# xin-pu/yolo-continuous

Measured on AMD Instinct MI355X. Metric: images/sec (whole node) + p50 end-to-end latency, 640×640 bs=32, 1/2/4/8 MI355X, higher is better.
Workload: dtype bf16; 1 GPU; yolov7 COCO-80 640x640, 32 images per GPU per step: forward + decode + NMS (+ all-gather); global_batch=32, per_gpu_batch=32, image_size=640, parallelism=dp1, hip_graph=True, mode=concurrent, batches_in_flight=3, max_det=300

## Files before the change

yolo-continuous_amd/csrc/ycx_misc.hip:

```cpp
#include <dlfcn.h>
#include <stdio.h>
#include <vector>

#include "ycx_internal.h"

namespace {

template <typename T>
struct Vec;
template <>
struct Vec<__bf16> {
  typedef bf16x8 type;
  static constexpr int N = 8;
};
template <>
struct Vec<_Float16> {
  typedef __attribute__((ext_vector_type(8))) _Float16 type;
  static constexpr int N = 8;
};
template <>
struct Vec<float> {
  typedef f32x4 type;
  static constexpr int N = 4;
};

template <typename T>
__global__ void __launch_bounds__(256) maxpool_kernel(ycx_pool_desc d, const T* __restrict__ x,
                                                      T* __restrict__ y) {
  typedef typename Vec<T>::type V;
  constexpr int VN = Vec<T>::N;
  const int cv = d.c / VN;
  const long long total = (long long)d.n * d.ho * d.wo * cv;
  for (long long i = blockIdx.x * (long long)blockDim.x + threadIdx.x; i < total;
       i += (long long)gridDim.x * blockDim.x) {
    int c = (int)(i % cv);
    long long p = i / cv;
    int ox = (int)(p % d.wo);
    long long t = p / d.wo;
    int oy = (int)(t % d.ho);
    int n = (int)(t / d.ho);
    float m[VN];
#pragma unroll
    for (int j = 0; j < VN; ++j) m[j] = -INFINITY;
    const int y0 = oy * d.stride - d.pad, x0 = ox * d.stride - d.pad;
    const int ya = max(y0, 0), yb = min(y0 + d.k, d.h), xa = max(x0, 0), xb = min(x0 + d.k, d.w);
    for (int iy = ya; iy < yb; ++iy)
      for (int ix = xa; ix < xb; ++ix) {
        V v = *reinterpret_cast<const V*>(x + (((size_t)n * d.h + iy) * d.w + ix) * d.in_c_stride +
                                          d.in_c_off + c * VN);
#pragma unroll
        for (int j = 0; j < VN; ++j) m[j] = ycx_pool_max(m[j], (float)v[j]);
      }
    V o;
#pragma unroll
    for (int j = 0; j < VN; ++j) o[j] = (T)m[j];
    *reinterpret_cast<V*>(y + (((size_t)n * d.ho + oy) * d.wo + ox) * d.out_c_stride + d.out_c_off +
                          c * VN) = o;
  }
}

template <typename T>
__global__ void __launch_bounds__(256) maxpool_rows_kernel(ycx_pool_desc d, const T* __restrict__ x,
                                                           T* __restrict__ y) {
  typedef typename Vec<T>::type V;
  constexpr int VN = Vec<T>::N;
  const int cv = d.c / VN;
  const int i = blockIdx.x * blockDim.x + threadIdx.x;
  if (i >= d.wo * cv) return;
  const int row = blockIdx.y, n = row / d.ho, oy = row - n * d.ho;
  const int ox = i / cv, c = i - ox * cv;
  float m[VN];
#pragma unroll
  for (int j = 0; j < VN; ++j) m[j] = -INFINITY;
  const int y0 = oy * d.stride - d.pad, x0 = ox * d.stride - d.pad;
  const int ya = max(y0, 0), yb = min(y0 + d.k, d.h), xa = max(x0, 0), xb = min(x0 + d.k, d.w);
  for (int iy = ya; iy < yb; ++iy) {
    const T* rowp = x + ((size_t)(n * d.h + iy) * d.w) * d.in_c_stride + d.in_c_off + c * VN;
    for (int ix = xa; ix < xb; ++ix) {
      const V v = *reinterpret_cast<const V*>(rowp + (size_t)ix * d.in_c_stride);
#pragma unroll
      for (int j = 0; j < VN; ++j) m[j] = ycx_pool_max(m[j], (float)v[j]);
    }
  }
  V o;
#pragma unroll
  for (int j = 0; j < VN; ++j) o[j] = (T)m[j];
  *reinterpret_cast<V*>(y + ((size_t)row * d.wo + ox) * d.out_c_stride + d.out_c_off + c * VN) = o;
}

template <typename T>
__global__ void __launch_bounds__(256) copy_kernel(ycx_copy_desc d, const T* __restrict__ x,
                                                   T* __restrict__ y) {
  typedef typename Vec<T>::type V;
  constexpr int VN = Vec<T>::N;
  const int cv = d.c / VN;
  const int ho = d.h * d.scale, wo = d.w * d.scale;
  const long long total = (long long)d.n * ho * wo * cv;
  for (long long i = blockIdx.x * (long long)blockDim.x + threadIdx.x; i < total;
       i += (long long)gridDim.x * blockDim.x) {
    int c = (int)(i % cv);
    long long p = i / cv;
    int ox = (int)(p % wo);
    long long t = p / wo;
    int oy = (int)(t % ho);
    int n = (int)(t / ho);
    int iy = oy / d.scale, ix = ox / d.scale;
    V v = *reinterpret_cast<const V*>(x + (((size_t)n * d.h + iy) * d.w + ix) * d.in_c_stride +
                                      d.in_c_off + c * VN);
    if (d.out_layout == YCX_OUT_NCHW_F32) {
      float* yf = reinterpret_cast<float*>(y);
#pragma unroll
      for (int j = 0; j < VN; ++j)
        yf[(((size_t)n * d.out_c_stride + d.out_c_off + c * VN + j) * ho + oy) * wo + ox] = (float)v[j];
    } else {
      *reinterpret_cast<V*>(y + (((size_t)n * ho + oy) * wo + ox) * d.out_c_stride + d.out_c_off + c * VN) = v;
    }
  }
}

__device__ __forceinline__ void f8x8_unpack(uint2 v, float f[8]) {
  f[0] = __builtin_amdgcn_cvt_f32_fp8((int)v.x, 0); f[1] = __builtin_amdgcn_cvt_f32_fp8((int)v.x, 1);
  f[2] = __builtin_amdgcn_cvt_f32_fp8((int)v.x, 2); f[3] = __builtin_amdgcn_cvt_f32_fp8((int)v.x, 3);
  f[4] = __builtin_amdgcn_cvt_f32_fp8((int)v.y, 0); f[5] = __builtin_amdgcn_cvt_f32_fp8((int)v.y, 1);
  f[6] = __builtin_amdgcn_cvt_f32_fp8((int)v.y, 2); f[7] = __builtin_amdgcn_cvt_f32_fp8((int)v.y, 3);
}
__device__ __forceinline__ uint32_t f8x4_pack_sat(float a, float b, float c, float d) {
  int w = __builtin_amdgcn_cvt_pk_fp8_f32(fminf(fmaxf(a, -448.f), 448.f), fminf(fmaxf(b, -448.f), 448.f), 0, false);
  w = __builtin_amdgcn_cvt_pk_fp8_f32(fminf(fmaxf(c, -448.f), 448.f), fminf(fmaxf(d, -448.f), 448.f), w, true);
  return (uint32_t)w;
}

__global__ void __launch_bounds__(256) maxpool_f8_kernel(ycx_pool_desc d, const uint8_t* __restrict__ x,
                                                         uint8_t* __restrict__ y) {
  const int cv = d.c / 8;
  const long long total = (long long)d.n * d.ho * d.wo * cv;
  for (long long i = blockIdx.x * (long long)blockDim.x + threadIdx.x; i < total;
       i += (long long)gridDim.x * blockDim.x) {
    int c = (int)(i % cv);
    long long p = i / cv;
    int ox = (int)(p % d.wo);
    long long t = p / d.wo;
    int oy = (int)(t % d.ho);
    int n = (int)(t / d.ho);
    float m[8], f[8];
#pragma unroll
    for (int j = 0; j < 8; ++j) m[j] = -INFINITY;
    const int y0 = oy * d.stride - d.pad, x0 = ox * d.stride - d.pad;
    const int ya = max(y0, 0), yb = min(y0 + d.k, d.h), xa = max(x0, 0), xb = min(x0 + d.k, d.w);
    for (int iy = ya; iy < yb; ++iy)
      for (int ix = xa; ix < xb; ++ix) {
        f8x8_unpack(*reinterpret_cast<const uint2*>(x + (((size_t)n * d.h + iy) * d.w + ix) * d.in_c_stride +
                                                    d.in_c_off + c * 8), f);
#pragma unroll
        for (int j = 0; j < 8; ++j) m[j] = fmaxf(m[j], f[j]);
      }
    *reinterpret_cast<uint2*>(y + (((size_t)n * d.ho + oy) * d.wo + ox) * d.out_c_stride + d.out_c_off + c * 8) =
        make_uint2(f8x4_pack_sat(m[0], m[1], m[2], m[3]), f8x4_pack_sat(m[4], m[5], m[6], m[7]));
  }
}

__global__ void __launch_bounds__(256) copy_f8_kernel(ycx_copy_desc d, const uint8_t* __restrict__ x,
                                                      uint8_t* __restrict__ y) {
  const int cv = d.c / 8;
  const int ho = d.h * d.scale, wo = d.w * d.scale;
  const long long total = (long long)d.n * ho * wo * cv;
  for (long long i = blockIdx.x * (long long)blockDim.x + threadIdx.x; i < total;
       i += (long long)gridDim.x * blockDim.x) {
    int c = (int)(i % cv);
    long long p = i / cv;
    int ox = (int)(p % wo);
    long long t = p / wo;
    int oy = (int)(t % ho);
    int n = (int)(t / ho);
    int iy = oy / d.scale, ix = ox / d.scale;
    const uint2 v = *reinterpret_cast<const uint2*>(x + (((size_t)n * d.h + iy) * d.w + ix) * d.in_c_stride +
                                                    d.in_c_off + c * 8);
    if (d.out_layout == YCX_OUT_NCHW_F32) {
      float f[8];
      f8x8_unpack(v, f);
      float* yf = reinterpret_cast<float*>(y);
#pragma unroll
      for (int j = 0; j < 8; ++j)
        yf[(((size_t)n * d.out_c_stride + d.out_c_off + c * 8 + j) * ho + oy) * wo + ox] = f[j] * d.dequant;
    } else {
      *reinterpret_cast<uint2*>(y + (((size_t)n * ho + oy) * wo + ox) * d.out_c_stride + d.out_c_off + c * 8) = v;
    }
  }
}

__global__ void __launch_bounds__(256) quantize_f8_kernel(const float* __restrict__ x, uint8_t* __restrict__ y,
                                                          long long n, float scale) {
  for (long long i = (blockIdx.x * (long long)blockDim.x + threadIdx.x) * 4; i < n;
       i += (long long)gridDim.x * blockDim.x * 4) {
    float v[4];
#pragma unroll
    for (int j = 0; j < 4; ++j) v[j] = i + j < n ? x[i + j] * scale : 0.0f;
    const uint32_t w = f8x4_pack_sat(v[0], v[1], v[2], v[3]);
#pragma unroll
    for (int j = 0; j < 4; ++j)
      if (i + j < n) y[i + j] = (uint8_t)(w >> (8 * j));
  }
}

template <int E>
__device__ __forceinline__ float pool_max_e(float a, float b) {
  if constexpr (E == 1) return fmaxf(a, b);
  else return ycx_pool_max(a, b);
}
template <int E, bool HALF = false>
__device__ __forceinline__ void chunk_to_f(uint4 v, float (&f)[16 / E]) {
  if constexpr (E == 2 && HALF) {
    const _Float16* b = reinterpret_cast<const _Float16*>(&v);
#pragma unroll
    for (int j = 0; j < 8; ++j) f[j] = (float)b[j];
  } else if constexpr (E == 2) {
    const __bf16* b = reinterpret_cast<const __bf16*>(&v);
#pragma unroll
    for (int j = 0; j < 8; ++j) f[j] = (float)b[j];
  } else {
    float* g = f;
    f8x8_unpack(make_uint2(v.x, v.y), g);
    f8x8_unpack(make_uint2(v.z, v.w), g + 8);
  }
}
template <int E, bool HALF = false>
__device__ __forceinline__ uint4 f_to_chunk(const float (&f)[16 / E]) {
  uint4 v;
  if constexpr (E == 2 && HALF) {
    _Float16* b = reinterpret_cast<_Float16*>(&v);
#pragma unroll
    for (int j = 0; j < 8; ++j) b[j] = (_Float16)f[j];
  } else if constexpr (E == 2) {
    __bf16* b = reinterpret_cast<__bf16*>(&v);
#pragma unroll
    for (int j = 0; j < 8; ++j) b[j] = (__bf16)f[j];
  } else {
    v.x = f8x4_pack_sat(f[0], f[1], f[2], f[3]);
    v.y = f8x4_pack_sat(f[4], f[5], f[6], f[7]);
    v.z = f8x4_pack_sat(f[8], f[9], f[10], f[11]);
    v.w = f8x4_pack_sat(f[12], f[13], f[14], f[15]);
  }
  return v;
}

template <int E, bool HALF = false>
__global__ void __launch_bounds__(256) maxpool_cascade_kernel(ycx_pool_desc d, int cc, const uint8_t* __restrict__ x,
                                                              uint8_t* __restrict__ y) {
  extern __shared__ uint4 lds_chunks[];
  constexpr int NE = 16 / E;
  const int H = d.h, W = d.w, HW = H * W, r = d.k / 2;
  const int nchunk = cc * E / 16;
  const int items = HW * nchunk;
  const int n = blockIdx.x / (d.c / cc), c0 = (blockIdx.x % (d.c / cc)) * cc;
  uint4* S = lds_chunks;
  uint4* T = lds_chunks + items;
  const size_t px0 = (size_t)n * HW;
  for (int i = threadIdx.x; i < items; i += blockDim.x) {
    const int pix = i / nchunk, g = i - pix * nchunk;
    S[i] = *reinterpret_cast<const uint4*>(x + ((px0 + pix) * d.in_c_stride + d.in_c_off + c0) * E + g * 16);
  }
  __syncthreads();
  for (int lv = 0; lv < d.levels; ++lv) {
    for (int i = threadIdx.x; i < items; i += blockDim.x) {
      const int pix = i / nchunk, g = i - pix * nchunk, yy = pix / W, xx = pix - yy * W;
      float m[NE], f[NE];
#pragma unroll
      for (int j = 0; j < NE; ++j) m[j] = -INFINITY;
      for (int xi = max(xx - r, 0); xi <= min(xx + r, W - 1); ++xi) {
        chunk_to_f<E, HALF>(S[(yy * W + xi) * nchunk + g], f);
#pragma unroll
        for (int j = 0; j < NE; ++j) m[j] = pool_max_e<E>(m[j], f[j]);
      }
      T[i] = f_to_chunk<E, HALF>(m);
    }
    __syncthreads();
    for (int i = threadIdx.x; i < items; i += blockDim.x) {
      const int pix = i / nchunk, g = i - pix * nchunk, yy = pix / W, xx = pix - yy * W;
      float m[NE], f[NE];
#pragma unroll
      for (int j = 0; j < NE; ++j) m[j] = -INFINITY;
      for (int yi = max(yy - r, 0); yi <= min(yy + r, H - 1); ++yi) {
        chunk_to_f<E, HALF>(T[(yi * W + xx) * nchunk + g], f);
#pragma unroll
        for (int j = 0; j < NE; ++j) m[j] = pool_max_e<E>(m[j], f[j]);
      }
      const uint4 v = f_to_chunk<E, HALF>(m);
      S[i] = v;
      *reinterpret_cast<uint4*>(y + ((px0 + pix) * d.out_c_stride + d.out_c_off + lv * d.c + c0) * E + g * 16) = v;
    }
    __syncthreads();
  }
}

unsigned grid_for(long long total) {
  long long b = (total + 255) / 256;
  if (b > 256LL * 16) b = 256LL * 16;
  return (unsigned)(b < 1 ? 1 : b);
}

}

extern "C" ycx_status ycx_maxpool(const ycx_pool_desc* d, const void* x, void* y, void* stream) {
  YCX_CHECK_ARG(d && x && y);
  YCX_CHECK_ARG(d->n > 0 && d->h > 0 && d->w > 0 && d->c > 0 && d->k > 0 && d->stride > 0 && d->pad >= 0);
  YCX_CHECK_ARG(d->ho == (d->h + 2 * d->pad - d->k) / d->stride + 1);
  YCX_CHECK_ARG(d->wo == (d->w + 2 * d->pad - d->k) / d->stride + 1);
  YCX_CHECK_ARG(d->pad * 2 <= d->k);
  YCX_CHECK_ARG(d->in_c_off + d->c <= d->in_c_stride && d->out_c_off + d->c <= d->out_c_stride);
  YCX_CHECK_SUPPORTED(d->dtype == YCX_DT_BF16 || d->dtype == YCX_DT_F32 || d->dtype == YCX_DT_FP8 ||
                      d->dtype == YCX_DT_F16);
  const int vn = d->dtype == YCX_DT_F32 ? 4 : 8;
  YCX_CHECK_SUPPORTED(d->c % vn == 0 && d->in_c_off % vn == 0 && d->in_c_stride % vn == 0 &&
                      d->out_c_off % vn == 0 && d->out_c_stride % vn == 0);
  hipStream_t st = reinterpret_cast<hipStream_t>(stream);
  const bool h16 = d->dtype == YCX_DT_F16;
  if (d->levels > 1) {
    YCX_CHECK_ARG(d->stride == 1 && d->k % 2 == 1 && d->pad == d->k / 2 && d->ho == d->h && d->wo == d->w);
    YCX_CHECK_ARG(d->out_c_off + d->levels * d->c <= d->out_c_stride);
    YCX_CHECK_SUPPORTED(d->dtype == YCX_DT_BF16 || d->dtype == YCX_DT_FP8 || h16);
    const int esz = d->dtype == YCX_DT_FP8 ? 1 : 2;
    const long long hw = (long long)d->h * d->w;
    int cc = 0;
    for (int t = 128; t * esz >= 16; t >>= 1)
      if (d->c % t == 0 && 2 * hw * t * esz <= 65536) { cc = t; break; }
    YCX_CHECK_SUPPORTED(cc > 0);
    const dim3 g((unsigned)(d->n * (d->c / cc)));
    const size_t lds = (size_t)(2 * hw * cc * esz);
    if (h16)
      hipLaunchKernelGGL((maxpool_cascade_kernel<2, true>), g, dim3(256), lds, st, *d, cc, (const uint8_t*)x,
                         (uint8_t*)y);
    else if (esz == 2)
      hipLaunchKernelGGL(maxpool_cascade_kernel<2>, g, dim3(256), lds, st, *d, cc, (const uint8_t*)x, (uint8_t*)y);
    else
      hipLaunchKernelGGL(maxpool_cascade_kernel<1>, g, dim3(256), lds, st, *d, cc, (const uint8_t*)x, (uint8_t*)y);
    return ycx_launch_status();
  }
  long long total = (long long)d->n * d->ho * d->wo * (d->c / vn);
  const long long rows = (long long)d->n * d->ho, rowlen = (long long)d->wo * (d->c / vn);
  if (d->dtype != YCX_DT_FP8 && rows <= 65535 && total < (1LL << 31) &&
      (long long)d->n * d->h * d->w * d->in_c_stride < (1LL << 31)) {
    const dim3 g((unsigned)((rowlen + 255) / 256), (unsigned)rows);
    if (h16)
      hipLaunchKernelGGL(maxpool_rows_kernel<_Float16>, g, dim3(256), 0, st, *d, (const _Float16*)x, (_Float16*)y);
    else if (d->dtype == YCX_DT_BF16)
      hipLaunchKernelGGL(maxpool_rows_kernel<__bf16>, g, dim3(256), 0, st, *d, (const __bf16*)x, (__bf16*)y);
    else
      hipLaunchKernelGGL(maxpool_rows_kernel<float>, g, dim3(256), 0, st, *d, (const float*)x, (float*)y);
    return ycx_launch_status();
  }
  if (d->dtype == YCX_DT_FP8)
    hipLaunchKernelGGL(maxpool_f8_kernel, dim3(grid_for(total)), dim3(256), 0, st, *d, (const uint8_t*)x,
                       (uint8_t*)y);
  else if (h16)
    hipLaunchKernelGGL(maxpool_kernel<_Float16>, dim3(grid_for(total)), dim3(256), 0, st, *d,
                       (const _Float16*)x, (_Float16*)y);
  else if (d->dtype == YCX_DT_BF16)
    hipLaunchKernelGGL(maxpool_kernel<__bf16>, dim3(grid_for(total)), dim3(256), 0, st, *d,
                       (const __bf16*)x, (__bf16*)y);
  else
    hipLaunchKernelGGL(maxpool_kernel<float>, dim3(grid_for(total)), dim3(256), 0, st, *d, (const float*)x,
                       (float*)y);
  return ycx_launch_status();
}

extern "C" ycx_status ycx_copy_channels(const ycx_copy_desc* d, const void* x, void* y, void* stream) {
  YCX_CHECK_ARG(d && x && y);
  YCX_CHECK_ARG(d->n > 0 && d->h > 0 && d->w > 0 && d->c > 0 && (d->scale == 1 || d->scale == 2));
  YCX_CHECK_ARG(d->in_c_off + d->c <= d->in_c_stride && d->out_c_off + d->c <= d->out_c_stride);
  YCX_CHECK_SUPPORTED(d->out_layout == YCX_OUT_NHWC || d->out_layout == YCX_OUT_NCHW_F32);
  YCX_CHECK_SUPPORTED(d->dtype == YCX_DT_BF16 || d->dtype == YCX_DT_F32 || d->dtype == YCX_DT_FP8 ||
                      d->dtype == YCX_DT_F16);
  const int vn = d->dtype == YCX_DT_F32 ? 4 : 8;
  YCX_CHECK_SUPPORTED(d->c % vn == 0 && d->in_c_off % vn == 0 && d->in_c_stride % vn == 0 &&
                      d->out_c_off % vn == 0 && d->out_c_stride % vn == 0);
  hipStream_t st = reinterpret_cast<hipStream_t>(stream);
  long long total = (long long)d->n * d->h * d->scale * d->w * d->scale * (d->c / vn);
  if (d->dtype == YCX_DT_FP8)
    hipLaunchKernelGGL(copy_f8_kernel, dim3(grid_for(total)), dim3(256), 0, st, *d, (const uint8_t*)x,
                       (uint8_t*)y);
  else if (d->dtype == YCX_DT_F16)
    hipLaunchKernelGGL(copy_kernel<_Float16>, dim3(grid_for(total)), dim3(256), 0, st, *d, (const _Float16*)x,
                       (_Float16*)y);
  else if (d->dtype == YCX_DT_BF16)
    hipLaunchKernelGGL(copy_kernel<__bf16>, dim3(grid_for(total)), dim3(256), 0, st, *d, (const __bf16*)x,
                       (__bf16*)y);
  else
    hipLaunchKernelGGL(copy_kernel<float>, dim3(grid_for(total)), dim3(256), 0, st, *d, (const float*)x,
                       (float*)y);
  return ycx_launch_status();
}

extern "C" ycx_status ycx_quantize_fp8(const float* x, void* y, int64_t n, float scale, void* stream) {
  YCX_CHECK_ARG(n >= 0 && (n == 0 || (x && y)));
  if (n == 0) return YCX_OK;
  hipLaunchKernelGGL(quantize_f8_kernel, dim3(grid_for((n + 3) / 4)), dim3(256), 0,
                     reinterpret_cast<hipStream_t>(stream), x, (uint8_t*)y, (long long)n, scale);
  return ycx_launch_status();
}

static_assert(sizeof(ycx_depth_desc) <= sizeof(ycx_conv_desc[2]), "ycx_depth_desc must not grow ycx_op's union");

static ycx_status run_one(const ycx_op& op, void* stream) {
  switch (op.kind) {
    case YCX_OP_CONV:
      return ycx_conv2d_ws(&op.d.conv, op.in, op.weight, op.bias, op.out, op.residual, op.workspace,
                           op.workspace ? ycx_conv_workspace_size(&op.d.conv) : 0, stream);
    case YCX_OP_STEM:
      return ycx_stem_conv(&op.d.conv, (const float*)op.in, (const float*)op.weight, op.bias, op.out, stream);
    case YCX_OP_STEM_REORG:
      return ycx_stem_conv_reorg(&op.d.conv, (const float*)op.in, (const float*)op.weight, op.bias, op.out, stream);
    case YCX_OP_GCONV:
      return ycx_conv2d_grouped(&op.d.conv, op.in, (const float*)op.weight, op.bias, op.out, op.residual,
                                stream);
    case YCX_OP_DECONV:
      return ycx_deconv2d(&op.d.conv, op.in, op.weight, op.bias, op.out, stream);
    case YCX_OP_GHOST:
      return ycx_ghost_dw(&op.d.conv, op.in, (const float*)op.weight, op.bias, op.out, op.residual, stream);
    case YCX_OP_POOL:
      return ycx_maxpool(&op.d.pool, op.in, op.out, stream);
    case YCX_OP_COPY:
      return ycx_copy_channels(&op.d.copy, op.in, op.out, stream);
    case YCX_OP_DEPTH:
      return ycx_space_depth(&op.d.depth, op.in, op.out, stream);
    case YCX_OP_STEM2:
      return ycx_stem_conv2(&op.d.pair[0], &op.d.pair[1], (const float*)op.in, (const float*)op.weight, op.bias,
                            op.weight2, op.bias2, op.out, stream);
    case YCX_OP_CONV_PAIR:
      if (op.out3)
        return ycx_conv2d_pair_pool(&op.d.pair[0], &op.d.pair[1], &op.conv3, op.in, op.weight, op.bias, op.out,
                                    op.weight2, op.bias2, op.out2, op.weight3, op.bias3, op.out3, stream);
      return ycx_conv2d_pair(&op.d.pair[0], &op.d.pair[1], op.in, op.weight, op.bias, op.out, op.weight2, op.bias2,
                             op.out2, stream);
    case YCX_OP_HEAD:
      return ycx_conv2d_head(&op.d.head.conv, &op.d.head.head, op.in, op.weight, op.bias, (float*)op.out,
                             (ycx_cand*)op.cand, op.cand_rows, op.cand_counts, op.status, stream);
    default:
      return YCX_ERR_BAD_ARG;
  }
}

static int g_trace = 0;
static int (*g_roctx_push)(const char*) = nullptr;
static int (*g_roctx_pop)() = nullptr;

extern "C" ycx_status ycx_set_trace(int32_t on) {
  if (!on) {
    g_trace = 0;
    return YCX_OK;
  }
  if (!g_roctx_push) {
    void* h = dlopen("librocprofiler-sdk-roctx.so.1", RTLD_NOW | RTLD_LOCAL);
    if (!h) h = dlopen("librocprofiler-sdk-roctx.so", RTLD_NOW | RTLD_LOCAL);
    if (!h) return YCX_ERR_UNSUPPORTED;
    auto push = reinterpret_cast<int (*)(const char*)>(dlsym(h, "roctxRangePushA"));
    auto pop = reinterpret_cast<int (*)()>(dlsym(h, "roctxRangePop"));
    if (!push || !pop) return YCX_ERR_UNSUPPORTED;
    g_roctx_pop = pop;
    g_roctx_push = push;
  }
  g_trace = 1;
  return YCX_OK;
}

static void trace_push(int32_t i, const ycx_op& op) {
  static const char* kinds[] = {"?", "conv", "stem", "pool", "copy", "stem2", "head", "conv_pair", "stem_reorg",
                                "gconv", "deconv", "ghost", "depth"};
  const char* k = (op.kind >= 1 && op.kind <= 12) ? kinds[op.kind] : kinds[0];
  char buf[160];
  if (op.kind == YCX_OP_CONV || op.kind == YCX_OP_STEM || op.kind == YCX_OP_HEAD || op.kind == YCX_OP_STEM2 ||
      op.kind == YCX_OP_CONV_PAIR || op.kind == YCX_OP_STEM_REORG || op.kind == YCX_OP_GCONV || op.kind == YCX_OP_DECONV ||
      op.kind == YCX_OP_GHOST) {
    const ycx_conv_desc& c = op.kind == YCX_OP_HEAD ? op.d.head.conv
                             : op.kind == YCX_OP_STEM2 || op.kind == YCX_OP_CONV_PAIR ? op.d.pair[1] : op.d.conv;
    snprintf(buf, sizeof buf, "op%d %s %s n%d %dx%d %d->%d k%d s%d", i, k,
             op.kind == YCX_OP_CONV ? ycx_conv_tile_name(c.tile ? c.tile : ycx_conv_pick_tile(&c)) : "", c.n, c.h,
             c.w, c.cin, c.cout, c.kh, c.stride);
  } else {
    snprintf(buf, sizeof buf, "op%d %s", i, k);
  }
  g_roctx_push(buf);
}

extern "C" ycx_status ycx_run_ops(const ycx_op* ops, int32_t n_ops, void* stream, void* const* events) {
  YCX_CHECK_ARG(ops && n_ops >= 0);
  hipStream_t st = reinterpret_cast<hipStream_t>(stream);
  for (int32_t i = 0; i < n_ops; ++i) {
    if (events && hipEventRecord(reinterpret_cast<hipEvent_t>(events[i]), st) != hipSuccess)
      return YCX_ERR_LAUNCH;
    if (g_trace) trace_push(i, ops[i]);
    ycx_status s = run_one(ops[i], stream);
    if (g_trace) g_roctx_pop();
    if (s != YCX_OK) return s;
  }
  if (events && hipEventRecord(reinterpret_cast<hipEvent_t>(events[n_ops]), st) != hipSuccess)
    return YCX_ERR_LAUNCH;
  return YCX_OK;
}

extern "C" ycx_status ycx_graph_capture(const ycx_op* ops, int32_t n_ops, void* stream, void** graph_exec) {
  YCX_CHECK_ARG(ops && graph_exec && stream);
  hipStream_t st = reinterpret_cast<hipStream_t>(stream);
  hipGraph_t g = nullptr;
  if (hipStreamBeginCapture(st, hipStreamCaptureModeThreadLocal) != hipSuccess) return YCX_ERR_LAUNCH;
  ycx_status s = ycx_run_ops(ops, n_ops, stream, nullptr);
  hipError_t e = hipStreamEndCapture(st, &g);
  if (s != YCX_OK) {
    if (g) (void)hipGraphDestroy(g);
    return s;
  }
  if (e != hipSuccess || !g) return YCX_ERR_LAUNCH;
  hipGraphExec_t ex = nullptr;
  e = hipGraphInstantiate(&ex, g, nullptr, nullptr, 0);
  (void)hipGraphDestroy(g);
  if (e != hipSuccess) return YCX_ERR_LAUNCH;
  *graph_exec = ex;
  return YCX_OK;
}

extern "C" ycx_status ycx_graph_launch(void* graph_exec, void* stream) {
  YCX_CHECK_ARG(graph_exec);
  return hipGraphLaunch(reinterpret_cast<hipGraphExec_t>(graph_exec), reinterpret_cast<hipStream_t>(stream)) ==
                 hipSuccess
             ? YCX_OK
             : YCX_ERR_LAUNCH;
}

extern "C" ycx_status ycx_graph_destroy(void* graph_exec) {
  YCX_CHECK_ARG(graph_exec);
  return hipGraphExecDestroy(reinterpret_cast<hipGraphExec_t>(graph_exec)) == hipSuccess ? YCX_OK
                                                                                         : YCX_ERR_LAUNCH;
}

#ifdef YCX_DEBUG_BOUNDS
extern "C" ycx_status ycx_dbg_bounds_conv(unsigned*, int);
extern "C" ycx_status ycx_dbg_bounds_conv_f16(unsigned*, int);
#endif

extern "C" ycx_status ycx_debug_bounds(uint32_t* out, int32_t reset) {
  YCX_CHECK_ARG(out);
  out[0] = out[1] = 0;
#ifdef YCX_DEBUG_BOUNDS
  ycx_status s = ycx_dbg_bounds_conv(out, reset);
  if (s == YCX_OK) s = ycx_dbg_bounds_conv_f16(out, reset);
  return s;
#else
  (void)reset;
  return YCX_ERR_UNSUPPORTED;
#endif
}

extern "C" int ycx_abi_version(void) { return YCX_ABI_VERSION; }

extern "C" size_t ycx_struct_size(int32_t which) {
  switch (which) {
    case 0: return sizeof(ycx_conv_desc);
    case 1: return sizeof(ycx_pool_desc);
    case 2: return sizeof(ycx_copy_desc);
    case 3: return sizeof(ycx_decode_desc);
    case 4: return sizeof(ycx_cand);
    case 5: return sizeof(ycx_filter_desc);
    case 6: return sizeof(ycx_decode_filter_desc);
    case 7: return sizeof(ycx_nms_desc);
    case 8: return sizeof(ycx_op);
    case 9: return sizeof(ycx_letterbox_desc);
    case 10: return sizeof(ycx_correct_desc);
    case 11: return sizeof(ycx_head_desc);
    default: return 0;
  }
}

extern "C" const char* ycx_strerror(ycx_status s) {
  switch (s) {
    case YCX_OK: return "ok";
    case YCX_ERR_BAD_ARG: return "ycx: bad argument (null pointer or inconsistent shape)";
    case YCX_ERR_UNSUPPORTED: return "ycx: unsupported shape/dtype for the HIP kernels";
    case YCX_ERR_LAUNCH: return "ycx: HIP launch/runtime failure";
    case YCX_ERR_CAPACITY: return "ycx: workspace or output capacity too small";
    default: return "ycx: unknown status";
  }
}
```

Measured before the change: 7205 images/s.

## Rewrite cascaded maxpool with packed integer order keys and sliding-window segments

The SPP cascaded maxpool kernel now encodes bf16/f16/fp8 values into order-preserving 16-bit integer keys and takes maxima with packed i16 max instead of converting to float and back. Each thread computes a segment of 4 outputs along a line with shared partial maxima, a van Herk style reuse, and the kernel is templated on radius for k=3/5/7. It also makes the channel slice smaller with more threads per block and unrolls the global loads. The goal is to cut ALU and LDS work in a small kernel. In exchange the encode/decode logic is more complex, and NaN handling has to stay correct.

```diff
diff --git a/yolo-continuous_amd/csrc/ycx_misc.hip b/yolo-continuous_amd/csrc/ycx_misc.hip
--- a/yolo-continuous_amd/csrc/ycx_misc.hip
+++ b/yolo-continuous_amd/csrc/ycx_misc.hip
@@ -1,5 +1,6 @@
 #include <dlfcn.h>
 #include <stdio.h>
+#include <algorithm>
 #include <vector>
 
 #include "ycx_internal.h"
@@ -202,93 +203,208 @@
   }
 }
 
-template <int E>
-__device__ __forceinline__ float pool_max_e(float a, float b) {
-  if constexpr (E == 1) return fmaxf(a, b);
-  else return ycx_pool_max(a, b);
-}
-template <int E, bool HALF = false>
-__device__ __forceinline__ void chunk_to_f(uint4 v, float (&f)[16 / E]) {
-  if constexpr (E == 2 && HALF) {
-    const _Float16* b = reinterpret_cast<const _Float16*>(&v);
-#pragma unroll
-    for (int j = 0; j < 8; ++j) f[j] = (float)b[j];
-  } else if constexpr (E == 2) {
-    const __bf16* b = reinterpret_cast<const __bf16*>(&v);
-#pragma unroll
-    for (int j = 0; j < 8; ++j) f[j] = (float)b[j];
+typedef short s16x2 __attribute__((ext_vector_type(2)));
+typedef unsigned short u16x2 __attribute__((ext_vector_type(2)));
+__device__ __forceinline__ uint32_t pk_max_i16(uint32_t a, uint32_t b) {
+  return __builtin_bit_cast(uint32_t, __builtin_elementwise_max(__builtin_bit_cast(s16x2, a), __builtin_bit_cast(s16x2, b)));
+}
+__device__ __forceinline__ uint32_t pk_min_u16(uint32_t a, uint32_t b) {
+  return __builtin_bit_cast(uint32_t, __builtin_elementwise_min(__builtin_bit_cast(u16x2, a), __builtin_bit_cast(u16x2, b)));
+}
+__device__ __forceinline__ uint32_t pk_add_u16(uint32_t a, uint32_t b) {
+  return __builtin_bit_cast(uint32_t, (u16x2)(__builtin_bit_cast(u16x2, a) + __builtin_bit_cast(u16x2, b)));
+}
+__device__ __forceinline__ uint32_t pk_sub_u16(uint32_t a, uint32_t b) {
+  return __builtin_bit_cast(uint32_t, (u16x2)(__builtin_bit_cast(u16x2, a) - __builtin_bit_cast(u16x2, b)));
+}
+__device__ __forceinline__ uint32_t pk_subsat_u16(uint32_t a, uint32_t b) {
+  return __builtin_bit_cast(uint32_t, __builtin_elementwise_sub_sat(__builtin_bit_cast(u16x2, a), __builtin_bit_cast(u16x2, b)));
+}
+__device__ __forceinline__ uint32_t pk_sign_i16(uint32_t a) {
+  return __builtin_bit_cast(uint32_t, (s16x2)(__builtin_bit_cast(s16x2, a) >> (s16x2)(15)));
+}
+
+constexpr uint32_t POOL_PAD = 0x80008000u;
+
+template <bool HALF>
+struct PoolKey16 {
+  static constexpr int E = 2, NW = 4;
+  static constexpr uint32_t ABS = 0x7FFF7FFFu, INF = HALF ? 0x7C007C00u : 0x7F807F80u, NNAN = ABS - INF;
+  static constexpr int QUIET = HALF ? 9 : 6;
+  static __device__ __forceinline__ uint32_t enc(uint32_t w) {
+    w |= pk_min_u16(pk_subsat_u16(w & ABS, INF), 0x00010001u) << QUIET;
+    return pk_sub_u16(w ^ (pk_sign_i16(w) & ABS), NNAN);
+  }
+  static __device__ __forceinline__ uint32_t dec(uint32_t k) {
+    k = pk_add_u16(k, NNAN);
+    return k ^ (pk_sign_i16(k) & ABS);
+  }
+  static __device__ __forceinline__ uint4 encode(uint4 v) { return make_uint4(enc(v.x), enc(v.y), enc(v.z), enc(v.w)); }
+  static __device__ __forceinline__ void expand(uint4 v, uint32_t (&r)[NW]) { r[0] = v.x; r[1] = v.y; r[2] = v.z; r[3] = v.w; }
+  static __device__ __forceinline__ uint4 compact(const uint32_t (&r)[NW]) { return make_uint4(r[0], r[1], r[2], r[3]); }
+  static __device__ __forceinline__ uint4 decode(const uint32_t (&r)[NW]) {
+    return make_uint4(dec(r[0]), dec(r[1]), dec(r[2]), dec(r[3]));
+  }
+};
+
+struct PoolKey8 {
+  static constexpr int E = 1, NW = 8;
+  static constexpr uint32_t HI = 0xFF00FF00u, MAG = 0x7F007F00u, ONE = 0x01000100u, LOWEST = 0x82008200u;
+  static __device__ __forceinline__ uint32_t enc(uint32_t v) { return pk_add_u16(v ^ (pk_sign_i16(v) & MAG), ONE); }
+  static __device__ __forceinline__ uint32_t dec(uint32_t k) {
+    k = pk_sub_u16(pk_max_i16(k, LOWEST), ONE);
+    return k ^ (pk_sign_i16(k) & MAG);
+  }
+  static __device__ __forceinline__ void expand(uint4 v, uint32_t (&r)[NW]) {
+    r[0] = (v.x << 8) & HI; r[1] = v.x & HI; r[2] = (v.y << 8) & HI; r[3] = v.y & HI;
+    r[4] = (v.z << 8) & HI; r[5] = v.z & HI; r[6] = (v.w << 8) & HI; r[7] = v.w & HI;
+  }
+  static __device__ __forceinline__ uint4 compact(const uint32_t (&r)[NW]) {
+    return make_uint4(r[1] | (r[0] >> 8), r[3] | (r[2] >> 8), r[5] | (r[4] >> 8), r[7] | (r[6] >> 8));
+  }
+  static __device__ __forceinline__ uint4 encode(uint4 v) {
+    uint32_t r[NW];
+    expand(v, r);
+#pragma unroll
+    for (int i = 0; i < NW; ++i) r[i] = enc(r[i]);
+    return compact(r);
+  }
+  static __device__ __forceinline__ uint4 decode(const uint32_t (&r)[NW]) {
+    uint32_t q[NW];
+#pragma unroll
+    for (int i = 0; i < NW; ++i) q[i] = dec(r[i]);
+    return compact(q);
+  }
+};
+
+constexpr int POOL_SEG = 4;
+constexpr int POOL_SLICE = 64;
+constexpr int POOL_THREADS = 512;
+
+template <int NW, int RAD, int SEG>
+__device__ __forceinline__ void pool_windows(const uint32_t (&a)[SEG + 2 * RAD][NW], uint32_t (&o)[SEG][NW]) {
+  static_assert(RAD >= 1 && RAD <= 3, "window radius");
+  constexpr int NA = SEG + 2 * RAD;
+#pragma unroll
+  for (int w = 0; w < NW; ++w) {
+    uint32_t p1[NA - 1], p2[NA - 3 > 0 ? NA - 3 : 1];
+#pragma unroll
+    for (int j = 0; j < NA - 1; ++j) p1[j] = pk_max_i16(a[j][w], a[j + 1][w]);
+    if constexpr (RAD >= 2) {
+#pragma unroll
+      for (int j = 0; j < NA - 3; ++j) p2[j] = pk_max_i16(p1[j], p1[j + 2]);
+    }
+#pragma unroll
+    for (int j = 0; j < SEG; ++j)
+      o[j][w] = RAD == 1 ? pk_max_i16(p1[j], a[j + 2][w]) : RAD == 2 ? pk_max_i16(p2[j], a[j + 4][w])
+                                                                      : pk_max_i16(p2[j], p2[j + 3]);
+  }
+}
+
+template <class K, int RAD>
+__device__ __forceinline__ void pool_line(const uint4* P, int base, int step, int t0, int len, int r,
+                                          uint32_t (&o)[POOL_SEG][K::NW]) {
+  constexpr int NW = K::NW, SEG = POOL_SEG;
+  if constexpr (RAD > 0) {
+    uint32_t a[SEG + 2 * RAD][NW];
+#pragma unroll
+    for (int j = 0; j < SEG + 2 * RAD; ++j) {
+      const int t = t0 - RAD + j;
+      if (t >= 0 && t < len) {
+        K::expand(P[base + t * step], a[j]);
+      } else {
+#pragma unroll
+        for (int w = 0; w < NW; ++w) a[j][w] = POOL_PAD;
+      }
+    }
+    pool_windows<NW, RAD, SEG>(a, o);
   } else {
-    float* g = f;
-    f8x8_unpack(make_uint2(v.x, v.y), g);
-    f8x8_unpack(make_uint2(v.z, v.w), g + 8);
-  }
-}
-template <int E, bool HALF = false>
-__device__ __forceinline__ uint4 f_to_chunk(const float (&f)[16 / E]) {
-  uint4 v;
-  if constexpr (E == 2 && HALF) {
-    _Float16* b = reinterpret_cast<_Float16*>(&v);
-#pragma unroll
-    for (int j = 0; j < 8; ++j) b[j] = (_Float16)f[j];
-  } else if constexpr (E == 2) {
-    __bf16* b = reinterpret_cast<__bf16*>(&v);
-#pragma unroll
-    for (int j = 0; j < 8; ++j) b[j] = (__bf16)f[j];
-  } else {
-    v.x = f8x4_pack_sat(f[0], f[1], f[2], f[3]);
-    v.y = f8x4_pack_sat(f[4], f[5], f[6], f[7]);
-    v.z = f8x4_pack_sat(f[8], f[9], f[10], f[11]);
-    v.w = f8x4_pack_sat(f[12], f[13], f[14], f[15]);
-  }
-  return v;
-}
-
-template <int E, bool HALF = false>
-__global__ void __launch_bounds__(256) maxpool_cascade_kernel(ycx_pool_desc d, int cc, const uint8_t* __restrict__ x,
-                                                              uint8_t* __restrict__ y) {
+#pragma unroll
+    for (int j = 0; j < SEG; ++j) {
+#pragma unroll
+      for (int w = 0; w < NW; ++w) o[j][w] = POOL_PAD;
+      if (t0 + j < len)
+        for (int t = max(t0 + j - r, 0); t <= min(t0 + j + r, len - 1); ++t) {
+          uint32_t f[NW];
+          K::expand(P[base + t * step], f);
+#pragma unroll
+          for (int w = 0; w < NW; ++w) o[j][w] = pk_max_i16(o[j][w], f[w]);
+        }
+    }
+  }
+}
+
+template <class K, int RAD>
+__global__ void __launch_bounds__(POOL_THREADS) pool_cascade_kernel(ycx_pool_desc d, int cs, const uint8_t* __restrict__ x,
+                                                                    uint8_t* __restrict__ y) {
   extern __shared__ uint4 lds_chunks[];
-  constexpr int NE = 16 / E;
+  constexpr int E = K::E, NW = K::NW, SEG = POOL_SEG;
   const int H = d.h, W = d.w, HW = H * W, r = d.k / 2;
-  const int nchunk = cc * E / 16;
-  const int items = HW * nchunk;
-  const int n = blockIdx.x / (d.c / cc), c0 = (blockIdx.x % (d.c / cc)) * cc;
+  const int nchunk = 1 << cs, WG = W << cs, items = HW << cs;
+  const int nslice = (d.c * E) >> (4 + cs);
+  const int n = blockIdx.x / nslice, sl = blockIdx.x - n * nslice;
+  const int tid = threadIdx.x, nthr = blockDim.x;
   uint4* S = lds_chunks;
   uint4* T = lds_chunks + items;
-  const size_t px0 = (size_t)n * HW;
-  for (int i = threadIdx.x; i < items; i += blockDim.x) {
-    const int pix = i / nchunk, g = i - pix * nchunk;
-    S[i] = *reinterpret_cast<const uint4*>(x + ((px0 + pix) * d.in_c_stride + d.in_c_off + c0) * E + g * 16);
+  const size_t in_px = (size_t)d.in_c_stride * E, out_px = (size_t)d.out_c_stride * E, level = (size_t)d.c * E;
+  const uint8_t* xs = x + ((size_t)n * HW * d.in_c_stride + d.in_c_off) * E + (size_t)sl * (16 << cs);
+  uint8_t* ys = y + ((size_t)n * HW * d.out_c_stride + d.out_c_off) * E + (size_t)sl * (16 << cs);
+
+  constexpr int U = 8;
+  for (int base = tid; base < items; base += U * nthr) {
+    uint4 v[U];
+#pragma unroll
+    for (int u = 0; u < U; ++u) {
+      const int i = base + u * nthr;
+      if (i < items) v[u] = *reinterpret_cast<const uint4*>(xs + (size_t)(i >> cs) * in_px + (i & (nchunk - 1)) * 16);
+    }
+#pragma unroll
+    for (int u = 0; u < U; ++u) {
+      const int i = base + u * nthr;
+      if (i < items) S[i] = K::encode(v[u]);
+    }
   }
   __syncthreads();
+
+  const int nsy = (H + SEG - 1) / SEG, nsx = (W + SEG - 1) / SEG;
   for (int lv = 0; lv < d.levels; ++lv) {
-    for (int i = threadIdx.x; i < items; i += blockDim.x) {
-      const int pix = i / nchunk, g = i - pix * nchunk, yy = pix / W, xx = pix - yy * W;
-      float m[NE], f[NE];
-#pragma unroll
-      for (int j = 0; j < NE; ++j) m[j] = -INFINITY;
-      for (int xi = max(xx - r, 0); xi <= min(xx + r, W - 1); ++xi) {
-        chunk_to_f<E, HALF>(S[(yy * W + xi) * nchunk + g], f);
-#pragma unroll
-        for (int j = 0; j < NE; ++j) m[j] = pool_max_e<E>(m[j], f[j]);
-      }
-      T[i] = f_to_chunk<E, HALF>(m);
+    for (int it = tid; it < nsy * WG; it += nthr) {
+      const int sy = it / WG, cg = it - sy * WG, y0 = sy * SEG;
+      uint32_t o[SEG][NW];
+      pool_line<K, RAD>(S, cg, WG, y0, H, r, o);
+#pragma unroll
+      for (int j = 0; j < SEG; ++j)
+        if (y0 + j < H) T[(y0 + j) * WG + cg] = K::compact(o[j]);
     }
     __syncthreads();
-    for (int i = threadIdx.x; i < items; i += blockDim.x) {
-      const int pix = i / nchunk, g = i - pix * nchunk, yy = pix / W, xx = pix - yy * W;
-      float m[NE], f[NE];
-#pragma unroll
-      for (int j = 0; j < NE; ++j) m[j] = -INFINITY;
-      for (int yi = max(yy - r, 0); yi <= min(yy + r, H - 1); ++yi) {
-        chunk_to_f<E, HALF>(T[(yi * W + xx) * nchunk + g], f);
-#pragma unroll
-        for (int j = 0; j < NE; ++j) m[j] = pool_max_e<E>(m[j], f[j]);
-      }
-      const uint4 v = f_to_chunk<E, HALF>(m);
-      S[i] = v;
-      *reinterpret_cast<uint4*>(y + ((px0 + pix) * d.out_c_stride + d.out_c_off + lv * d.c + c0) * E + g * 16) = v;
-    }
-    __syncthreads();
+    const bool more = lv + 1 < d.levels;
+    for (int it = tid; it < (H * nsx) << cs; it += nthr) {
+      const int g = it & (nchunk - 1), t = it >> cs, yy = t / nsx, x0 = (t - yy * nsx) * SEG;
+      uint32_t o[SEG][NW];
+      pool_line<K, RAD>(T, ((yy * W) << cs) + g, nchunk, x0, W, r, o);
+#pragma unroll
+      for (int j = 0; j < SEG; ++j)
+        if (x0 + j < W) {
+          const int p = yy * W + x0 + j;
+          *reinterpret_cast<uint4*>(ys + p * out_px + lv * level + g * 16) = K::decode(o[j]);
+          if (more) S[(p << cs) + g] = K::compact(o[j]);
+        }
+    }
+    if (more) __syncthreads();
+  }
+}
+
+template <class K>
+void launch_pool_cascade(const ycx_pool_desc& d, int cs, unsigned threads, size_t lds, hipStream_t st, const void* x,
+                         void* y) {
+  const dim3 g((unsigned)(d.n * ((d.c * K::E) >> (4 + cs)))), b(threads);
+  const uint8_t* xb = (const uint8_t*)x;
+  uint8_t* yb = (uint8_t*)y;
+  switch (d.k) {
+    case 3: hipLaunchKernelGGL((pool_cascade_kernel<K, 1>), g, b, lds, st, d, cs, xb, yb); break;
+    case 5: hipLaunchKernelGGL((pool_cascade_kernel<K, 2>), g, b, lds, st, d, cs, xb, yb); break;
+    case 7: hipLaunchKernelGGL((pool_cascade_kernel<K, 3>), g, b, lds, st, d, cs, xb, yb); break;
+    default: hipLaunchKernelGGL((pool_cascade_kernel<K, 0>), g, b, lds, st, d, cs, xb, yb); break;
   }
 }
 
@@ -320,19 +436,20 @@
     YCX_CHECK_SUPPORTED(d->dtype == YCX_DT_BF16 || d->dtype == YCX_DT_FP8 || h16);
     const int esz = d->dtype == YCX_DT_FP8 ? 1 : 2;
     const long long hw = (long long)d->h * d->w;
-    int cc = 0;
-    for (int t = 128; t * esz >= 16; t >>= 1)
-      if (d->c % t == 0 && 2 * hw * t * esz <= 65536) { cc = t; break; }
-    YCX_CHECK_SUPPORTED(cc > 0);
-    const dim3 g((unsigned)(d->n * (d->c / cc)));
-    const size_t lds = (size_t)(2 * hw * cc * esz);
+    int cs = -1;
+    for (int t = 0; (16 << t) <= POOL_SLICE; ++t)
+      if ((d->c * esz) % (16 << t) == 0 && 2 * hw * (16 << t) <= 65536) cs = t;
+    YCX_CHECK_SUPPORTED(cs >= 0);
+    const size_t lds = (size_t)(2 * hw * (16 << cs));
+    const long long seg_h = (d->h + POOL_SEG - 1) / POOL_SEG, seg_w = (d->w + POOL_SEG - 1) / POOL_SEG;
+    const long long lanes = std::max(seg_h * d->w, seg_w * d->h) << cs;
+    const unsigned threads = (unsigned)std::min<long long>(POOL_THREADS, (lanes + 63) / 64 * 64);
     if (h16)
-      hipLaunchKernelGGL((maxpool_cascade_kernel<2, true>), g, dim3(256), lds, st, *d, cc, (const uint8_t*)x,
-                         (uint8_t*)y);
+      launch_pool_cascade<PoolKey16<true>>(*d, cs, threads, lds, st, x, y);
     else if (esz == 2)
-      hipLaunchKernelGGL(maxpool_cascade_kernel<2>, g, dim3(256), lds, st, *d, cc, (const uint8_t*)x, (uint8_t*)y);
+      launch_pool_cascade<PoolKey16<false>>(*d, cs, threads, lds, st, x, y);
     else
-      hipLaunchKernelGGL(maxpool_cascade_kernel<1>, g, dim3(256), lds, st, *d, cc, (const uint8_t*)x, (uint8_t*)y);
+      launch_pool_cascade<PoolKey8>(*d, cs, threads, lds, st, x, y);
     return ycx_launch_status();
   }
   long long total = (long long)d->n * d->ho * d->wo * (d->c / vn);
```

New measurement: 7219 images/s, median of 5. Within noise of the previous version (+0.2%).
